# robertknight/ocrs

Measured on AMD Instinct MI355X. Metric: pages/sec end-to-end (1024x1024), higher is better.
Workload: dtype f32

## Files before the change

### ocrs_amd/csrc/kernels_rec.hip

```cpp
#include <algorithm>

#include "common.hpp"
#include "kernels.hpp"
#include "split_mfma.hpp"

namespace ocrs {
namespace k {

typedef float f32x16 __attribute__((ext_vector_type(16)));
typedef unsigned u32x4 __attribute__((ext_vector_type(4)));
typedef float f32x4 __attribute__((ext_vector_type(4)));
typedef float f32x2 __attribute__((ext_vector_type(2)));
typedef unsigned u32x2 __attribute__((ext_vector_type(2)));
typedef __bf16 bf16x8 __attribute__((ext_vector_type(8)));
typedef __bf16 bf16x2 __attribute__((ext_vector_type(2)));

__device__ __forceinline__ int xcd_remap(int b, int nwg) {
    const int xcd = b & 7, q = nwg >> 3, r = nwg & 7;
    return (xcd < r ? xcd * (q + 1) : r * (q + 1) + (xcd - r) * q) + (b >> 3);
}

__device__ __forceinline__ int find_group(const int32_t* __restrict__ toff, int G, int tile) {
    int lo = 0, hi = G;
    while (hi - lo > 1) {
        int mid = (lo + hi) >> 1;
        if (toff[mid] <= tile) lo = mid; else hi = mid;
    }
    return lo;
}

__global__ void __launch_bounds__(256)
conv1_relu_pool_ragged_kernel(const float* __restrict__ x, RaggedView in, const float* __restrict__ wt,
                              const float* __restrict__ bias, int cout, float* __restrict__ y, RaggedView out) {
    __shared__ float sw[9 * 64 + 64];
    for (int i = threadIdx.x; i < 9 * cout; i += 256) sw[i] = wt[i];
    for (int i = threadIdx.x; i < cout; i += 256) sw[9 * 64 + i] = bias[i];
    __syncthreads();
    const int g = find_group(out.toff256, out.G, blockIdx.x);
    const int tile = blockIdx.x - out.toff256[g];
    const int ow = out.W[g], oh = out.H, iw = in.W[g], ih = in.H;
    const int64_t rows = (int64_t)out.n[g] * oh * ow;
    const float* __restrict__ xg = x + in.poff[g];
    float* __restrict__ yg = y + out.poff[g] * cout;
    const int cq = cout >> 2;
    const int step_px = 256 / cq;
    const int q = threadIdx.x % cq;
    int64_t r = (int64_t)tile * 256 + threadIdx.x / cq;
    int ox = (int)(r % ow);
    int64_t t0 = r / ow;
    int oy = (int)(t0 % oh);
    int64_t img = t0 / oh;
    float wq[9][4], bq[4];
#pragma unroll
    for (int t = 0; t < 9; t++)
#pragma unroll
        for (int c = 0; c < 4; c++) wq[t][c] = sw[t * cout + 4 * q + c];
#pragma unroll
    for (int c = 0; c < 4; c++) bq[c] = sw[9 * 64 + 4 * q + c];
    for (int it = 0; it < cq; it++, r += step_px) {
        if (r >= rows) break;
        if (it > 0) {
            ox += step_px;
            while (ox >= ow) { ox -= ow; if (++oy == oh) { oy = 0; img++; } }
        }
        const float* xi = xg + img * ih * iw;
        float p[4][4];
        const int iy0 = 2 * oy - 1, ix0 = 2 * ox - 1;
        if (iy0 >= 0 && iy0 + 3 < ih && ix0 >= 0 && ix0 + 3 < iw) {
            const float* pp = xi + (int64_t)iy0 * iw + ix0;
#pragma unroll
            for (int a = 0; a < 4; a++)
#pragma unroll
                for (int b = 0; b < 4; b++) p[a][b] = pp[a * iw + b];
        } else {
#pragma unroll
            for (int a = 0; a < 4; a++)
#pragma unroll
                for (int b = 0; b < 4; b++) {
                    const int iy = iy0 + a, ix = ix0 + b;
                    p[a][b] = ((unsigned)iy < (unsigned)ih && (unsigned)ix < (unsigned)iw) ? xi[(int64_t)iy * iw + ix] : 0.0f;
                }
        }
        float m[4];
#pragma unroll
        for (int py = 0; py < 2; py++)
#pragma unroll
            for (int px = 0; px < 2; px++) {
                float acc[4];
#pragma unroll
                for (int c = 0; c < 4; c++) acc[c] = bq[c];
#pragma unroll
                for (int ky = 0; ky < 3; ky++)
#pragma unroll
                    for (int kx = 0; kx < 3; kx++) {
                        const float xv = p[py + ky][px + kx];
#pragma unroll
                        for (int c = 0; c < 4; c++) acc[c] = fmaf(xv, wq[ky * 3 + kx][c], acc[c]);
                    }
#pragma unroll
                for (int c = 0; c < 4; c++) {
                    float v = acc[c] > 0.0f ? acc[c] : 0.0f;
                    if (py == 0 && px == 0) m[c] = v;
                    else m[c] = v > m[c] ? v : m[c];
                }
            }
        *reinterpret_cast<float4*>(yg + r * cout + 4 * q) = make_float4(m[0], m[1], m[2], m[3]);
    }
}

void conv1_relu_pool_ragged(const float* x, const RaggedView& in, const float* wt, const float* bias, int cout,
                            float* y, const RaggedView& out, hipStream_t s) {
    if (out.ntiles256 <= 0) return;
    hipLaunchKernelGGL(conv1_relu_pool_ragged_kernel, dim3(out.ntiles256), dim3(256), 0, s, x, in, wt, bias, cout, y, out);
}

template <bool AVG>
__global__ void __launch_bounds__(256)
pool_ragged_kernel(const float* __restrict__ x, RaggedView in, int c, int kh, int kw, float* __restrict__ y,
                   RaggedView out) {
    const int g = find_group(out.toff256, out.G, blockIdx.x);
    const int tile = blockIdx.x - out.toff256[g];
    const int ow = out.W[g], oh = out.H, iw = in.W[g], ih = in.H;
    const int64_t rows = (int64_t)out.n[g] * oh * ow;
    const float* __restrict__ xg = x + in.poff[g] * c;
    float* __restrict__ yg = y + out.poff[g] * c;
    const int cq = c >> 2;
    const float inv = 1.0f / (float)(kh * kw);
    for (int i = threadIdx.x; i < 256 * cq; i += 256) {
        const int64_t r = (int64_t)tile * 256 + i / cq;
        if (r >= rows) break;
        const int q = i % cq;
        const int ox = (int)(r % ow);
        const int oy = (int)((r / ow) % oh);
        const int64_t img = r / ((int64_t)ow * oh);
        const float* xp = xg + ((img * ih + (int64_t)oy * kh) * iw + (int64_t)ox * kw) * c + 4 * q;
        float4 acc = AVG ? make_float4(0.f, 0.f, 0.f, 0.f) : *reinterpret_cast<const float4*>(xp);
        for (int ky = 0; ky < kh; ky++)
            for (int kx = 0; kx < kw; kx++) {
                const float4 v = *reinterpret_cast<const float4*>(xp + ((int64_t)ky * iw + kx) * c);
                if (AVG) { acc.x = acc.x + v.x; acc.y = acc.y + v.y; acc.z = acc.z + v.z; acc.w = acc.w + v.w; }
                else {
                    acc.x = v.x > acc.x ? v.x : acc.x; acc.y = v.y > acc.y ? v.y : acc.y;
                    acc.z = v.z > acc.z ? v.z : acc.z; acc.w = v.w > acc.w ? v.w : acc.w;
                }
            }
        if (AVG) { acc.x = acc.x * inv; acc.y = acc.y * inv; acc.z = acc.z * inv; acc.w = acc.w * inv; }
        *reinterpret_cast<float4*>(yg + r * c + 4 * q) = acc;
    }
}

void pool_ragged(const float* x, const RaggedView& in, int c, int kh, int kw, bool avg, float* y, const RaggedView& out,
                 hipStream_t s) {
    if (out.ntiles256 <= 0) return;
    if (avg) hipLaunchKernelGGL((pool_ragged_kernel<true>), dim3(out.ntiles256), dim3(256), 0, s, x, in, c, kh, kw, y, out);
    else hipLaunchKernelGGL((pool_ragged_kernel<false>), dim3(out.ntiles256), dim3(256), 0, s, x, in, c, kh, kw, y, out);
}

__global__ void __launch_bounds__(256)
to_seq_packed_ragged_kernel(const float* __restrict__ x, RaggedView in, int c, const int32_t* __restrict__ pos,
                            const int32_t* __restrict__ off, float* __restrict__ y) {
    const int g = find_group(in.toff256, in.G, blockIdx.x);
    const int tile = blockIdx.x - in.toff256[g];
    const int T = in.W[g];
    const int64_t rows = (int64_t)in.n[g] * T;
    const float* __restrict__ xg = x + in.poff[g] * c;
    const int32_t* __restrict__ posg = pos + in.loff[g];
    const int cq = c >> 2;
    for (int i = threadIdx.x; i < 256 * cq; i += 256) {
        const int64_t r = (int64_t)tile * 256 + i / cq;
        if (r >= rows) break;
        const int q = i % cq;
        const int t = (int)(r % T);
        const int line = (int)(r / T);
        const float4 v = *reinterpret_cast<const float4*>(xg + r * c + 4 * q);
        *reinterpret_cast<float4*>(y + ((int64_t)off[t] + posg[line]) * c + 4 * q) = v;
    }
}

__global__ void __launch_bounds__(256)
avgpool_to_seq_ragged_kernel(const float* __restrict__ x, RaggedView in, RaggedView seq, int c,
                             const int32_t* __restrict__ pos, const int32_t* __restrict__ off, float* __restrict__ y) {
    const int g = find_group(seq.toff256, seq.G, blockIdx.x);
    const int tile = blockIdx.x - seq.toff256[g];
    const int T = seq.W[g], ih = in.H;
    const int64_t rows = (int64_t)seq.n[g] * T;
    const float* __restrict__ xg = x + in.poff[g] * c;
    const int32_t* __restrict__ posg = pos + seq.loff[g];
    const int cq = c >> 2;
    const float inv = 1.0f / (float)ih;
    for (int i = threadIdx.x; i < 256 * cq; i += 256) {
        const int64_t r = (int64_t)tile * 256 + i / cq;
        if (r >= rows) break;
        const int q = i % cq;
        const int t = (int)(r % T);
        const int64_t line = r / T;
        const float* xp = xg + (line * ih * T + t) * c + 4 * q;
        float4 acc = make_float4(0.f, 0.f, 0.f, 0.f);
        for (int ky = 0; ky < ih; ky++) {
            const float4 v = *reinterpret_cast<const float4*>(xp + (int64_t)ky * T * c);
            acc.x = acc.x + v.x; acc.y = acc.y + v.y; acc.z = acc.z + v.z; acc.w = acc.w + v.w;
        }
        acc.x = acc.x * inv; acc.y = acc.y * inv; acc.z = acc.z * inv; acc.w = acc.w * inv;
        *reinterpret_cast<float4*>(y + ((int64_t)off[t] + posg[line]) * c + 4 * q) = acc;
    }
}

void avgpool_to_seq_ragged(const float* x, const RaggedView& in, const RaggedView& seq, int c, const int32_t* d_pos,
                           const int32_t* d_off, float* y, hipStream_t s) {
    if (seq.ntiles256 <= 0) return;
    hipLaunchKernelGGL(avgpool_to_seq_ragged_kernel, dim3(seq.ntiles256), dim3(256), 0, s, x, in, seq, c, d_pos, d_off, y);
}

void to_seq_packed_ragged(const float* x, const RaggedView& in, int c, const int32_t* d_pos, const int32_t* d_off,
                          float* y, hipStream_t s) {
    if (in.ntiles256 <= 0) return;
    hipLaunchKernelGGL(to_seq_packed_ragged_kernel, dim3(in.ntiles256), dim3(256), 0, s, x, in, c, d_pos, d_off, y);
}

constexpr int RG_BM = 128, RG_BK = 16, RG_LDA = RG_BM + 1;
constexpr int CONV_WAVES = 4;
template <int BN, int TW, int PH, int PW, bool FLAT, int SPLIT = 0>
__global__ void __launch_bounds__(256, SPLIT == 3 ? 2 : SPLIT == 2 ? 3 : CONV_WAVES)
conv3x3_ragged_kernel(const float* __restrict__ X, RaggedView rv, int cin, const float* __restrict__ Bw,
                      const float* __restrict__ bias, int cout, int relu, float* __restrict__ Y,
                      const int64_t* __restrict__ out_poff) {
    extern __shared__ __attribute__((aligned(16))) float lds[];
    constexpr int NTW = BN / 64;
    constexpr int TH = RG_BM / TW;
    static_assert(TW == 32 || TW == 16, "patch width");
    static_assert(!SPLIT || (BN == 128 && RG_BK == 16), "split mode: 128-column blocks, 16-deep chunks");
    constexpr int NP = SPLIT ? SPLIT : 1;
    constexpr int SP_PLANE = split::PLANE;
    float* As = lds;
    float* Bs = lds + (SPLIT ? 2 * NP * SP_PLANE : 2 * RG_BK * RG_LDA);
    const int tid = threadIdx.x, lane = tid & 63, wave = tid >> 6;
    const int half = lane >> 5, l31 = lane & 31;
    const int wm = wave >> 1, wn = wave & 1;
    const int gtile = xcd_remap(blockIdx.x, gridDim.x);
    const int32_t* __restrict__ toff = FLAT ? (PW == 2 ? rv.toff2d_flat2 : rv.toff2d_flat) : rv.toff2d;
    const int g = find_group(toff, rv.G, gtile);
    const int tile = gtile - toff[g];
    const int H = rv.H, W = rv.W[g];
    const int tiles_h = H / TH;
    const int Wp = FLAT ? (PW == 2 ? (W + 1) & ~1 : W) : W;
    const int nimg = FLAT ? rv.n[g] : 1;
    int rb, img, x0, span = 1;
    if (FLAT) {
        rb = tile % tiles_h;
        const int c0 = (tile / tiles_h) * TW;
        img = c0 / Wp;
        x0 = c0 - img * Wp;
        span = min(nimg - img, (x0 + TW - 1) / Wp + 1);
    } else {
        const int tiles_w = (W + TW - 1) / TW;
        const int cb = tile % tiles_w;
        const int t2 = tile / tiles_w;
        rb = t2 % tiles_h;
        img = t2 / tiles_h;
        x0 = cb * TW;
    }
    const int y0 = rb * TH;
    const int n0 = blockIdx.y * BN;
    const float* __restrict__ A = X + (rv.poff[g] + (int64_t)img * H * W) * cin;
    const int K = 9 * cin;

    constexpr int AQ = RG_BK / 4;
    constexpr int AROWS = 256 / AQ;
    constexpr int AV = RG_BM / AROWS;
    const int ar = tid / AQ, akq = tid % AQ;
    int aoff[AV];
    unsigned amask[AV];
#pragma unroll
    for (int j = 0; j < AV; j++) {
        const int m = ar + AROWS * j;
        const int py = y0 + m / TW;
        int px = x0 + m % TW, ir = 0;
        if (FLAT) {
#pragma unroll
            for (int q = 0; q < 3; q++) { const bool nx = px >= Wp; px -= nx ? Wp : 0; ir += nx; }
        }
        unsigned mk = 0;
        if (px < W && ir < span) {
#pragma unroll
            for (int t9 = 0; t9 < 9; t9++) {
                const int iy = py + t9 / 3 - 1, ix = px + t9 % 3 - 1;
                if ((unsigned)iy < (unsigned)H && (unsigned)ix < (unsigned)W) mk |= 1u << t9;
            }
        }
        amask[j] = mk;
        aoff[j] = ((min(ir, span - 1) * H + py) * W + min(px, W - 1)) * cin + akq * 4;
    }
    constexpr int BV = RG_BK * BN / 4 / 256;
    f32x4 pa0[AV], pa1[AV];
    const uint64_t a_addr = reinterpret_cast<uint64_t>(A);
    const float* a_uniform = reinterpret_cast<const float*>(((uint64_t)(uint32_t)__builtin_amdgcn_readfirstlane((int)(a_addr >> 32)) << 32) |
                                                            (uint32_t)__builtin_amdgcn_readfirstlane((int)a_addr));
    const __amdgpu_buffer_rsrc_t a_rsrc = __builtin_amdgcn_make_buffer_rsrc(
        const_cast<float*>(a_uniform),  0,
        __builtin_amdgcn_readfirstlane((int)((int64_t)span * H * W * cin * sizeof(float))), 0x00020000);
    constexpr int OOB = 0x40000000;
    auto load_a_into = [&](int k0, f32x4 (&d0)[AV], f32x4 (&d1)[AV]) {
        const int tap = k0 / cin;
        const int ci0 = k0 - tap * cin;
        const int ky = tap / 3, kx = tap - ky * 3;
        const int delta = ((ky - 1) * W + (kx - 1)) * cin + ci0;
#pragma unroll
        for (int j = 0; j < AV; j++) {
            const int voff = ((amask[j] >> tap) & 1u) ? (aoff[j] + delta) * 4 : OOB;
            const u32x4 v0 = __builtin_amdgcn_raw_buffer_load_b128(a_rsrc, voff, 0, 0);
            const u32x4 v1 = __builtin_amdgcn_raw_buffer_load_b128(a_rsrc, voff + RG_BK * 4, 0, 0);
            d0[j] = __builtin_bit_cast(f32x4, v0);
            d1[j] = __builtin_bit_cast(f32x4, v1);
        }
    };
    auto load_a_pair = [&](int k0) { load_a_into(k0, pa0, pa1); };
    int boff[BV];
#pragma unroll
    for (int j = 0; j < BV; j++) {
        const int idx = tid + 256 * j;
        const int kk = idx / (BN / 4), nn = (idx % (BN / 4)) * 4;
        boff[j] = kk * cout + min(n0 + nn, cout - 4);
    }
    auto load_b = [&](int k0, int buf) {
        if constexpr (SPLIT != 0) {
            split::load_weights<NP>(Bw + ((int64_t)blockIdx.y * (K / RG_BK) + k0 / RG_BK) * split::image_floats,
                                    Bs + buf * NP * SP_PLANE, wave, lane);
            return;
        }
        const float* __restrict__ bk = Bw + (int64_t)k0 * cout;
        float* bdst = Bs + buf * RG_BK * BN + wave * 256;
#pragma unroll
        for (int j = 0; j < BV; j++)
            __builtin_amdgcn_global_load_lds((const __attribute__((address_space(1))) void*)(bk + boff[j]),
                                             (__attribute__((address_space(3))) void*)(bdst + 1024 * j), 16, 0, 0);
    };
    auto commit = [&](int buf, const f32x4 (&pa)[AV]) {
        if constexpr (SPLIT != 0) {
            char* base = reinterpret_cast<char*>(As + buf * NP * SP_PLANE);
#pragma unroll
            for (int j = 0; j < AV; j++) split::commit4<NP>(base, ar + AROWS * j, akq, pa[j][0], pa[j][1], pa[j][2], pa[j][3]);
            return;
        }
        float* a = As + buf * RG_BK * RG_LDA;
#pragma unroll
        for (int j = 0; j < AV; j++) {
            const int r = ar + AROWS * j;
            a[(akq * 4 + 0) * RG_LDA + r] = pa[j].x;
            a[(akq * 4 + 1) * RG_LDA + r] = pa[j].y;
            a[(akq * 4 + 2) * RG_LDA + r] = pa[j].z;
            a[(akq * 4 + 3) * RG_LDA + r] = pa[j].w;
        }
    };

    f32x16 acc[2][NTW];
#pragma unroll
    for (int t = 0; t < NTW; t++) {
        const int col = n0 + wn * (BN / 2) + t * 32 + l31;
        const float bv = col < cout ? bias[col] : 0.0f;
#pragma unroll
        for (int r = 0; r < 16; r++) { acc[0][t][r] = bv; acc[1][t][r] = bv; }
    }
    auto compute = [&](int buf, int bbuf = -1) {
        if constexpr (SPLIT != 0) {
            split::mma_chunk<NP>(reinterpret_cast<const char*>(As + buf * NP * SP_PLANE),
                                 reinterpret_cast<const char*>(Bs + (bbuf < 0 ? buf : bbuf) * NP * SP_PLANE), wm, wn, l31, half, acc);
            return;
        }
        const float* a = As + buf * RG_BK * RG_LDA + wm * 64 + l31;
        const float* b = Bs + buf * RG_BK * BN + wn * (BN / 2) + l31;
#pragma unroll
        for (int kp = 0; kp < RG_BK / 2; kp++) {
            const int kr = 2 * kp + half;
            const float a0 = a[kr * RG_LDA], a1 = a[kr * RG_LDA + 32];
#pragma unroll
            for (int t = 0; t < NTW; t++) {
                const float bt = b[kr * BN + t * 32];
                acc[0][t] = __builtin_amdgcn_mfma_f32_32x32x2f32(a0, bt, acc[0][t], 0, 0, 0);
                acc[1][t] = __builtin_amdgcn_mfma_f32_32x32x2f32(a1, bt, acc[1][t], 0, 0, 0);
            }
        }
    };
    const int nchunks = K / RG_BK;
    if constexpr (SPLIT != 0) {
        static_assert(AV == 2, "split::pipeline counts four activation loads per chunk pair");
        split::pipeline<NP>(nchunks,
                            [&](int k0, f32x4 (&d0)[AV], f32x4 (&d1)[AV]) { load_a_into(k0, d0, d1); },
                            [&](int k0, int ring) { load_b(k0, ring); },
                            [&](int abuf, const f32x4 (&d)[AV]) { commit(abuf, d); },
                            [&](int abuf, int ring) { compute(abuf, ring); });
    } else {
    load_a_pair(0);
    load_b(0, 0);
    commit(0, pa0);
    __syncthreads();
    for (int c = 0; c < nchunks; c += 2) {
        load_b((c + 1) * RG_BK, 1);
        compute(0);
        commit(1, pa1);
        __syncthreads();
        const bool more = c + 2 < nchunks;
        if (more) {
            load_a_pair((c + 2) * RG_BK);
            load_b((c + 2) * RG_BK, 0);
        }
        compute(1);
        if (more) commit(0, pa0);
        __syncthreads();
    }
    }

    const int Ho = H / PH, Wo = W / PW;
    float* __restrict__ C = Y + (out_poff[g] + (int64_t)img * Ho * Wo) * cout;
    auto act = [&](float v) { return relu ? (v > 0.0f ? v : 0.0f) : v; };
    if (PH == 1 && PW == 1 && n0 + BN <= cout && (cout & 3) == 0 && (((uintptr_t)Y) & 15) == 0) {
        constexpr int WN = BN / 2, LPR = WN / 4, RPI = 64 / LPR, NIT = 32 / RPI;
        static_assert(SPLIT != 0 || 4 * 32 * WN <= 2 * RG_BK * RG_LDA + 2 * RG_BK * BN, "staging must fit the operand tiles");
        float* stage = lds + wave * (32 * WN);
        const int srow = lane / LPR, sc4 = (lane % LPR) * 4;
        int soff[NIT];
#pragma unroll
        for (int it = 0; it < NIT; it++) {
            const int q = it * RPI + srow;
            int x = x0 + (TW == 32 ? q : (q & 15)), ir = 0;
            if (FLAT) {
#pragma unroll
                for (int k = 0; k < 3; k++) { const bool nx = x >= Wp; x -= nx ? Wp : 0; ir += nx; }
            }
            soff[it] = (x < W && (!FLAT || ir < span)) ? ((FLAT ? ir * Ho * Wo : 0) + x) * cout + n0 + wn * WN + sc4 : -1;
        }
#pragma unroll
        for (int i = 0; i < 2; i++) {
#pragma unroll
            for (int t = 0; t < NTW; t++)
#pragma unroll
                for (int r = 0; r < 16; r++)
                    stage[((r & 3) + 8 * (r >> 2) + 4 * half) * WN + t * 32 + l31] = act(acc[i][t][r]);
            asm volatile("s_waitcnt lgkmcnt(0)" ::: "memory");
#pragma unroll
            for (int it = 0; it < NIT; it++) {
                const int q = it * RPI + srow;
                if (soff[it] < 0) continue;
                const int ty = TW == 32 ? 2 * wm + i : 4 * wm + 2 * i + (q >> 4);
                *reinterpret_cast<f32x4*>(&C[soff[it] + (y0 + ty) * Wo * cout]) = *reinterpret_cast<const f32x4*>(&stage[q * WN + sc4]);
            }
            asm volatile("s_waitcnt lgkmcnt(0)" ::: "memory");
        }
        return;
    }
    constexpr int NX = TW == 16 ? 8 : 16;
    int xo_off[FLAT ? NX : 1];
    if (FLAT) {
#pragma unroll
        for (int jx = 0; jx < NX; jx++) {
            if (PW == 2 && (jx & 1)) { xo_off[jx] = -1; continue; }
            const int q = (jx & 3) + 8 * (jx >> 2) + 4 * half;
            int x = x0 + (TW == 32 ? q : (q & 15)), ir = 0;
#pragma unroll
            for (int k = 0; k < 3; k++) { const bool nx = x >= Wp; x -= nx ? Wp : 0; ir += nx; }
            xo_off[jx] = (x + (PW - 1) < W && ir < span) ? (ir * Ho * Wo + x / PW) * cout : -1;
        }
    }
#pragma unroll
    for (int t = 0; t < NTW; t++) {
        const int col = n0 + wn * (BN / 2) + t * 32 + l31;
        if (col >= cout) continue;
#pragma unroll
        for (int i = 0; i < 2; i++) {
            if (PH == 2 && TW == 32 && i == 1) continue;
#pragma unroll
            for (int r = 0; r < 16; r++) {
                if (PH == 2 && TW == 16 && (r & 8)) continue;
                if (PW == 2 && (r & 1)) continue;
                const int q = (r & 3) + 8 * (r >> 2) + 4 * half;
                const int ty = TW == 32 ? 2 * wm + i : 4 * wm + 2 * i + (r >> 3);
                const int tx = TW == 32 ? q : (q & 15);
                const int x = x0 + tx;
                if (FLAT ? xo_off[TW == 16 ? (r & 7) : r] < 0 : x + (PW - 1) >= W) continue;
                constexpr int VI = (PH == 2 && TW == 32) ? 1 : 0;
                constexpr int VR = (PH == 2 && TW == 16) ? 8 : 0;
                float m = act(acc[i][t][r]);
                if (PW == 2) { const float v = act(acc[i][t][(r + 1) & 15]); m = v > m ? v : m; }
                if (PH == 2) {
                    { const float v = act(acc[(i + VI) & 1][t][(r + VR) & 15]); m = v > m ? v : m; }
                    if (PW == 2) { const float v = act(acc[(i + VI) & 1][t][(r + VR + 1) & 15]); m = v > m ? v : m; }
                }
                const int yo = (y0 + ty) / PH;
                if (FLAT) C[xo_off[TW == 16 ? (r & 7) : r] + yo * Wo * cout + col] = m;
                else C[((int64_t)yo * Wo + x / PW) * cout + col] = m;
            }
        }
    }
}

constexpr int F12_MID = 32, F12_COUT = 64, F12_TW = 16, F12_TH = 8, F12_HW = F12_TW + 2, F12_HH = F12_TH + 2;
constexpr int F12_NPOS = F12_HH * F12_HW;
constexpr int F12_LD = F12_MID + 1;
constexpr int F12_BK = 16;
constexpr size_t F12_LDS = (size_t)(F12_NPOS * F12_LD + 2 * F12_BK * F12_COUT) * sizeof(float);

__global__ void __launch_bounds__(256, CONV_WAVES)
conv12_fused_kernel(const float* __restrict__ X0, RaggedView in0, RaggedView mid, const float* __restrict__ w1,
                    const float* __restrict__ b1, const float* __restrict__ Bw, const float* __restrict__ bias,
                    float* __restrict__ Y, const int64_t* __restrict__ out_poff) {
    extern __shared__ __attribute__((aligned(16))) float lds[];
    constexpr int BN = F12_COUT, TW = F12_TW, TH = F12_TH, LD = F12_LD;
    float* T = lds;
    float* Bs = lds + F12_NPOS * LD;
    const int tid = threadIdx.x, lane = tid & 63, wave = tid >> 6;
    const int half = lane >> 5, l31 = lane & 31;
    const int wm = wave >> 1, wn = wave & 1;
    const int gtile = xcd_remap(blockIdx.x, gridDim.x);
    const int g = find_group(mid.toff2d_gap, mid.G, gtile);
    const int tile = gtile - mid.toff2d_gap[g];
    const int H = mid.H, W = mid.W[g];
    const int H0 = in0.H, W0 = in0.W[g];
    const int tiles_h = H / TH;
    const int Wg = (W + 2) & ~1;
    const int nimg = mid.n[g];
    const int rb = tile % tiles_h;
    const int c0 = (tile / tiles_h) * TW;
    const int img = c0 / Wg;
    const int x0 = c0 - img * Wg;
    const int span = min(nimg - img, (x0 + TW - 1) / Wg + 1);
    const int y0 = rb * TH;

    constexpr int BV = F12_BK * BN / 4 / 256;
    const int boff = (tid / (BN / 4)) * BN + (tid % (BN / 4)) * 4;
    auto load_b = [&](int k0, int buf) {
#pragma unroll
        for (int j = 0; j < BV; j++)
            __builtin_amdgcn_global_load_lds((const __attribute__((address_space(1))) void*)(Bw + (int64_t)(k0 + 16 * j) * BN + boff),
                                             (__attribute__((address_space(3))) void*)(Bs + buf * F12_BK * BN + wave * 256 + 1024 * j), 16, 0, 0);
    };
    load_b(0, 0);

    {
        const int q = tid & 7;
        f32x2 wq[9][2], bq[2];
#pragma unroll
        for (int t = 0; t < 9; t++)
#pragma unroll
            for (int c = 0; c < 2; c++) wq[t][c] = f32x2{w1[t * F12_MID + 4 * q + 2 * c], w1[t * F12_MID + 4 * q + 2 * c + 1]};
#pragma unroll
        for (int c = 0; c < 2; c++) bq[c] = f32x2{b1[4 * q + 2 * c], b1[4 * q + 2 * c + 1]};
        const float* __restrict__ xg = X0 + in0.poff[g];
        for (int p = tid >> 3; p < F12_NPOS; p += 32) {
            const int hy = p / F12_HW, hx = p - hy * F12_HW;
            const int y = y0 - 1 + hy;
            int x = x0 - 1 + hx, ir = 0;
#pragma unroll
            for (int k = 0; k < 3; k++) { const bool nx = x >= Wg; x -= nx ? Wg : 0; ir += nx; }
            f32x2 m[2] = {f32x2{0.0f, 0.0f}, f32x2{0.0f, 0.0f}};
            if ((unsigned)y < (unsigned)H && x >= 0 && x < W && ir < span) {
                const float* xi = xg + (int64_t)(img + ir) * H0 * W0;
                float pt[4][4];
                const int iy0 = 2 * y - 1, ix0 = 2 * x - 1;
                if (iy0 >= 0 && iy0 + 3 < H0 && ix0 >= 0 && ix0 + 3 < W0) {
                    const float* pp = xi + (int64_t)iy0 * W0 + ix0;
#pragma unroll
                    for (int a = 0; a < 4; a++)
#pragma unroll
                        for (int b = 0; b < 4; b++) pt[a][b] = pp[a * W0 + b];
                } else {
#pragma unroll
                    for (int a = 0; a < 4; a++)
#pragma unroll
                        for (int b = 0; b < 4; b++) {
                            const int iy = iy0 + a, ix = ix0 + b;
                            pt[a][b] = ((unsigned)iy < (unsigned)H0 && (unsigned)ix < (unsigned)W0) ? xi[(int64_t)iy * W0 + ix] : 0.0f;
                        }
                }
#pragma unroll
                for (int py = 0; py < 2; py++)
#pragma unroll
                    for (int px = 0; px < 2; px++) {
                        f32x2 acc[2] = {bq[0], bq[1]};
#pragma unroll
                        for (int ky = 0; ky < 3; ky++)
#pragma unroll
                            for (int kx = 0; kx < 3; kx++) {
                                const float xs = pt[py + ky][px + kx];
                                const f32x2 xv = f32x2{xs, xs};
#pragma unroll
                                for (int c = 0; c < 2; c++) acc[c] = __builtin_elementwise_fma(xv, wq[ky * 3 + kx][c], acc[c]);
                            }
#pragma unroll
                        for (int c = 0; c < 2; c++) m[c] = (py == 0 && px == 0) ? acc[c] : __builtin_elementwise_max(acc[c], m[c]);
                    }
#pragma unroll
                for (int c = 0; c < 2; c++) {
                    m[c].x = m[c].x > 0.0f ? m[c].x : 0.0f;
                    m[c].y = m[c].y > 0.0f ? m[c].y : 0.0f;
                }
            }
            float* t = T + p * LD + 4 * q;
            t[0] = m[0].x; t[1] = m[0].y; t[2] = m[1].x; t[3] = m[1].y;
        }
    }

    f32x16 acc[2];
    {
        const int col = wn * 32 + l31;
        const float bv = bias[col];
#pragma unroll
        for (int r = 0; r < 16; r++) { acc[0][r] = bv; acc[1][r] = bv; }
    }
    int abase[2];
#pragma unroll
    for (int i = 0; i < 2; i++) {
        const int m = wm * 64 + i * 32 + l31;
        abase[i] = ((m / TW) * F12_HW + (m % TW)) * LD + half;
    }
    __syncthreads();
    constexpr int NCH = 9 * F12_MID / F12_BK;
    static_assert(F12_MID % F12_BK == 0 && F12_BK % 16 == 0, "chunk size");
#pragma unroll
    for (int c = 0; c < NCH; c++) {
        if (c + 1 < NCH) load_b((c + 1) * F12_BK, (c + 1) & 1);
        const int tap = (c * F12_BK) / F12_MID, ch0 = (c * F12_BK) % F12_MID;
        const int toff = ((tap / 3) * F12_HW + tap % 3) * LD + ch0;
        const float* b = Bs + (c & 1) * F12_BK * BN + wn * 32 + l31;
#pragma unroll
        for (int kp = 0; kp < F12_BK / 2; kp++) {
            const float a0 = T[abase[0] + toff + 2 * kp], a1 = T[abase[1] + toff + 2 * kp];
            const float bt = b[(2 * kp + half) * BN];
            acc[0] = __builtin_amdgcn_mfma_f32_32x32x2f32(a0, bt, acc[0], 0, 0, 0);
            acc[1] = __builtin_amdgcn_mfma_f32_32x32x2f32(a1, bt, acc[1], 0, 0, 0);
        }
        __syncthreads();
    }

    const int Ho = H / 2, Wo = W / 2;
    float* __restrict__ C = Y + (out_poff[g] + (int64_t)img * Ho * Wo) * BN;
    auto act = [&](float v) { return v > 0.0f ? v : 0.0f; };
    const int col = wn * 32 + l31;
    int xo_off[8];
#pragma unroll
    for (int jx = 0; jx < 8; jx++) {
        if (jx & 1) { xo_off[jx] = -1; continue; }
        int x = x0 + (jx & 3) + 8 * (jx >> 2) + 4 * half, ir = 0;
#pragma unroll
        for (int k = 0; k < 3; k++) { const bool nx = x >= Wg; x -= nx ? Wg : 0; ir += nx; }
        xo_off[jx] = (x + 1 < W && ir < span) ? (ir * Ho * Wo + x / 2) * BN : -1;
    }
#pragma unroll
    for (int i = 0; i < 2; i++)
#pragma unroll
        for (int r = 0; r < 8; r += 2) {
            if (xo_off[r & 7] < 0) continue;
            const float m = act(__builtin_fmaxf(__builtin_fmaxf(acc[i][r], acc[i][r + 1]), __builtin_fmaxf(acc[i][r + 8], acc[i][r + 9])));
            const int yo = (y0 + 4 * wm + 2 * i) / 2;
            C[xo_off[r & 7] + yo * Wo * BN + col] = m;
        }
}

constexpr int F12S_RS = 20;
constexpr int F12S_TILE = F12_HH * F12S_RS * 64;
constexpr int F12S_BTAP = F12_COUT * 64;
constexpr size_t f12s_lds(int np) { return (size_t)np * (F12S_TILE + 3 * F12S_BTAP); }

template <int NP>
__global__ void __launch_bounds__(256, NP == 3 ? 2 : 3)
conv12_fused_split_kernel(const float* __restrict__ X0, RaggedView in0, RaggedView mid, const float* __restrict__ w1,
                          const float* __restrict__ b1, const uint16_t* __restrict__ Bimg, const float* __restrict__ bias,
                          float* __restrict__ Y, const int64_t* __restrict__ out_poff) {
    extern __shared__ __attribute__((aligned(16))) float lds[];
    constexpr int BN = F12_COUT, TW = F12_TW, TH = F12_TH;
    char* T = reinterpret_cast<char*>(lds);
    char* Bs = T + NP * F12S_TILE;
    const int tid = threadIdx.x, lane = tid & 63, wave = tid >> 6;
    const int half = lane >> 5, l31 = lane & 31;
    const int wm = wave >> 1, wn = wave & 1;
    const int gtile = xcd_remap(blockIdx.x, gridDim.x);
    const int g = find_group(mid.toff2d_gap, mid.G, gtile);
    const int tile = gtile - mid.toff2d_gap[g];
    const int H = mid.H, W = mid.W[g];
    const int H0 = in0.H, W0 = in0.W[g];
    const int tiles_h = H / TH;
    const int Wg = (W + 2) & ~1;
    const int nimg = mid.n[g];
    const int rb = tile % tiles_h;
    const int c0 = (tile / tiles_h) * TW;
    const int img = c0 / Wg;
    const int x0 = c0 - img * Wg;
    const int span = min(nimg - img, (x0 + TW - 1) / Wg + 1);
    const int y0 = rb * TH;

    auto load_b = [&](int tap) {
        const char* src = reinterpret_cast<const char*>(Bimg) + (size_t)tap * 3 * F12S_BTAP;
        char* dst = Bs + (tap % 3) * NP * F12S_BTAP;
#pragma unroll
        for (int p = 0; p < NP; p++)
            __builtin_amdgcn_global_load_lds((const __attribute__((address_space(1))) void*)(src + p * F12S_BTAP + wave * 1024 + lane * 16),
                                             (__attribute__((address_space(3))) void*)(dst + p * F12S_BTAP + wave * 1024), 16, 0, 0);
    };
    load_b(0);
    load_b(1);

    {
        const int q = tid & 7;
        f32x2 wq[9][2], bq[2];
#pragma unroll
        for (int t = 0; t < 9; t++)
#pragma unroll
            for (int c = 0; c < 2; c++) wq[t][c] = f32x2{w1[t * F12_MID + 4 * q + 2 * c], w1[t * F12_MID + 4 * q + 2 * c + 1]};
#pragma unroll
        for (int c = 0; c < 2; c++) bq[c] = f32x2{b1[4 * q + 2 * c], b1[4 * q + 2 * c + 1]};
        const float* __restrict__ xg = X0 + in0.poff[g];
        auto cut = [](float a, float b) { return __builtin_bit_cast(unsigned, __builtin_convertvector(f32x2{a, b}, bf16x2)); };
        auto lo_f = [](unsigned pk) { return __uint_as_float(pk << 16); };
        auto hi_f = [](unsigned pk) { return __uint_as_float(pk & 0xFFFF0000u); };
        for (int p = tid >> 3; p < F12_NPOS; p += 32) {
            const int hy = p / F12_HW, hx = p - hy * F12_HW;
            const int y = y0 - 1 + hy;
            int x = x0 - 1 + hx, ir = 0;
#pragma unroll
            for (int k = 0; k < 3; k++) { const bool nx = x >= Wg; x -= nx ? Wg : 0; ir += nx; }
            f32x2 m[2] = {f32x2{0.0f, 0.0f}, f32x2{0.0f, 0.0f}};
            if ((unsigned)y < (unsigned)H && x >= 0 && x < W && ir < span) {
                const float* xi = xg + (int64_t)(img + ir) * H0 * W0;
                float pt[4][4];
                const int iy0 = 2 * y - 1, ix0 = 2 * x - 1;
                if (iy0 >= 0 && iy0 + 3 < H0 && ix0 >= 0 && ix0 + 3 < W0) {
                    const float* pp = xi + (int64_t)iy0 * W0 + ix0;
#pragma unroll
                    for (int a = 0; a < 4; a++)
#pragma unroll
                        for (int b = 0; b < 4; b++) pt[a][b] = pp[a * W0 + b];
                } else {
#pragma unroll
                    for (int a = 0; a < 4; a++)
#pragma unroll
                        for (int b = 0; b < 4; b++) {
                            const int iy = iy0 + a, ix = ix0 + b;
                            pt[a][b] = ((unsigned)iy < (unsigned)H0 && (unsigned)ix < (unsigned)W0) ? xi[(int64_t)iy * W0 + ix] : 0.0f;
                        }
                }
#pragma unroll
                for (int py = 0; py < 2; py++)
#pragma unroll
                    for (int px = 0; px < 2; px++) {
                        f32x2 acc[2] = {bq[0], bq[1]};
#pragma unroll
                        for (int ky = 0; ky < 3; ky++)
#pragma unroll
                            for (int kx = 0; kx < 3; kx++) {
                                const float xs = pt[py + ky][px + kx];
                                const f32x2 xv = f32x2{xs, xs};
#pragma unroll
                                for (int c = 0; c < 2; c++) acc[c] = __builtin_elementwise_fma(xv, wq[ky * 3 + kx][c], acc[c]);
                            }
#pragma unroll
                        for (int c = 0; c < 2; c++) m[c] = (py == 0 && px == 0) ? acc[c] : __builtin_elementwise_max(acc[c], m[c]);
                    }
#pragma unroll
                for (int c = 0; c < 2; c++) {
                    m[c].x = m[c].x > 0.0f ? m[c].x : 0.0f;
                    m[c].y = m[c].y > 0.0f ? m[c].y : 0.0f;
                }
            }
            const int off = (hy * F12S_RS + hx) * 64 + ((((q >> 1) ^ (hx >> 2)) & 3) << 4) + ((q & 1) << 3);
            u32x2 ph = {cut(m[0].x, m[0].y), cut(m[1].x, m[1].y)};
            const float r0 = m[0].x - lo_f(ph[0]), r1 = m[0].y - hi_f(ph[0]), r2 = m[1].x - lo_f(ph[1]), r3 = m[1].y - hi_f(ph[1]);
            u32x2 pm = {cut(r0, r1), cut(r2, r3)};
            *reinterpret_cast<u32x2*>(T + off) = ph;
            *reinterpret_cast<u32x2*>(T + F12S_TILE + off) = pm;
            if (NP == 3) {
                u32x2 pl = {cut(r0 - lo_f(pm[0]), r1 - hi_f(pm[0])), cut(r2 - lo_f(pm[1]), r3 - hi_f(pm[1]))};
                *reinterpret_cast<u32x2*>(T + 2 * F12S_TILE + off) = pl;
            }
        }
    }

    f32x16 acc[2];
    {
        const float bv = bias[wn * 32 + l31];
#pragma unroll
        for (int r = 0; r < 16; r++) { acc[0][r] = bv; acc[1][r] = bv; }
    }
    const int mx = l31 & 15;
    int pos0[2];
#pragma unroll
    for (int i = 0; i < 2; i++) {
        const int m = wm * 64 + i * 32 + l31;
        pos0[i] = (m / TW) * F12S_RS + mx;
    }
    const int nb = wn * 32 + l31;
    const int boff = nb * 64, bsw = (nb >> 2) & 3;
    asm volatile("" ::: "memory");
    __builtin_amdgcn_s_waitcnt(0x0070);
    __builtin_amdgcn_s_barrier();
    asm volatile("" ::: "memory");
#pragma unroll
    for (int tap = 0; tap < 9; tap++) {
        if (tap + 2 < 9) load_b(tap + 2);
        const int ky = tap / 3, kx = tap % 3;
        const int asw = ((mx + kx) >> 2) & 3;
        const char* bb = Bs + (tap % 3) * NP * F12S_BTAP + boff;
#pragma unroll
        for (int s2 = 0; s2 < 2; s2++) {
            const int qa = (((2 * s2 + half) ^ asw) & 3) << 4, qb = (((2 * s2 + half) ^ bsw) & 3) << 4;
            bf16x8 af[2][3], bfr[3];
#pragma unroll
            for (int i = 0; i < 2; i++)
#pragma unroll
                for (int p = 0; p < NP; p++) af[i][p] = *reinterpret_cast<const bf16x8*>(T + p * F12S_TILE + (pos0[i] + ky * F12S_RS + kx) * 64 + qa);
#pragma unroll
            for (int p = 0; p < NP; p++) bfr[p] = *reinterpret_cast<const bf16x8*>(bb + p * F12S_BTAP + qb);
#define OCRS_TERM12(PA, PB)                                                                                   \
            OCRS_SPLIT_MMA(af[0][PA], bfr[PB], acc[0]);                                                       \
            OCRS_SPLIT_MMA(af[1][PA], bfr[PB], acc[1]);
            if (NP == 3) { OCRS_TERM12(NP - 1, 0) OCRS_TERM12(0, NP - 1) OCRS_TERM12(1, 1) }
            OCRS_TERM12(1, 0) OCRS_TERM12(0, 1) OCRS_TERM12(0, 0)
#undef OCRS_TERM12
        }
        asm volatile("" ::: "memory");
        if (tap + 2 < 9) __builtin_amdgcn_s_waitcnt(0x0070 | NP);
        else __builtin_amdgcn_s_waitcnt(0x0070);
        __builtin_amdgcn_s_barrier();
        asm volatile("" ::: "memory");
    }

    const int Ho = H / 2, Wo = W / 2;
    float* __restrict__ C = Y + (out_poff[g] + (int64_t)img * Ho * Wo) * BN;
    auto act = [&](float v) { return v > 0.0f ? v : 0.0f; };
    const int col = wn * 32 + l31;
    int xo_off[8];
#pragma unroll
    for (int jx = 0; jx < 8; jx++) {
        if (jx & 1) { xo_off[jx] = -1; continue; }
        int x = x0 + (jx & 3) + 8 * (jx >> 2) + 4 * half, ir = 0;
#pragma unroll
        for (int k = 0; k < 3; k++) { const bool nx = x >= Wg; x -= nx ? Wg : 0; ir += nx; }
        xo_off[jx] = (x + 1 < W && ir < span) ? (ir * Ho * Wo + x / 2) * BN : -1;
    }
#pragma unroll
    for (int i = 0; i < 2; i++)
#pragma unroll
        for (int r = 0; r < 8; r += 2) {
            if (xo_off[r & 7] < 0) continue;
            const float m = act(__builtin_fmaxf(__builtin_fmaxf(acc[i][r], acc[i][r + 1]), __builtin_fmaxf(acc[i][r + 8], acc[i][r + 9])));
            const int yo = (y0 + 4 * wm + 2 * i) / 2;
            C[xo_off[r & 7] + yo * Wo * BN + col] = m;
        }
}

void conv12_split_weights(const float* w, std::vector<uint16_t>* out) {
    out->assign((size_t)9 * 3 * F12_COUT * 32, 0);
    auto bits = [](float f) { uint32_t u; memcpy(&u, &f, 4); return u; };
    auto from = [](uint32_t u) { float f; memcpy(&f, &u, 4); return f; };
    auto rne = [&](float f) { const uint32_t u = bits(f); return (u + 0x7FFFu + ((u >> 16) & 1u)) >> 16; };
    for (int tap = 0; tap < 9; tap++)
        for (int n = 0; n < F12_COUT; n++)
            for (int k = 0; k < 32; k++) {
                const float x = w[(size_t)(tap * 32 + k) * F12_COUT + n];
                const uint32_t hb = rne(x);
                const float r1 = x - from(hb << 16);
                const uint32_t mb = rne(r1);
                const uint32_t lb = rne(r1 - from(mb << 16));
                const size_t e = (size_t)n * 32 + (size_t)((((k >> 3) ^ (n >> 2)) & 3) * 8) + (k & 7);
                uint16_t* img = out->data() + (size_t)tap * 3 * F12_COUT * 32;
                img[e] = (uint16_t)hb;
                img[F12_COUT * 32 + e] = (uint16_t)mb;
                img[2 * F12_COUT * 32 + e] = (uint16_t)lb;
            }
}

bool conv12_fused_ragged(const float* x, const RaggedView& in0, const RaggedView& mid, const float* w1, const float* b1,
                         int c1, const float* w2, const float* b2, int c2, float* y, const RaggedView& out, hipStream_t s,
                         const uint16_t* w2split) {
    if (option(OPT_CONV12_FUSE) == 0) return false;
    if (c1 != F12_MID || c2 != F12_COUT || mid.H % F12_TH != 0 || in0.H != 2 * mid.H || out.H * 2 != mid.H) return false;
    if (mid.min_w < 11 || mid.ntiles2d_gap <= 0) return false;
    if (mid.max_tile_px_ * 4 * (int64_t)sizeof(float) >= (int64_t)1 << 30 ||
        mid.max_tile_px_ * F12_COUT * (int64_t)sizeof(float) >= (int64_t)1 << 30) return false;
    if (!x) return true;
    const int numerics = option(OPT_NUMERICS);
    if (numerics != 0 && w2split) {
        static std::atomic<uint64_t> ok3{0}, ok2{0};
        if (numerics == 2) {
            allow_dynamic_lds(reinterpret_cast<const void*>(&conv12_fused_split_kernel<2>), ok2);
            hipLaunchKernelGGL((conv12_fused_split_kernel<2>), dim3(mid.ntiles2d_gap), dim3(256), f12s_lds(2), s, x, in0, mid, w1, b1, w2split, b2, y, out.poff);
        } else {
            allow_dynamic_lds(reinterpret_cast<const void*>(&conv12_fused_split_kernel<3>), ok3);
            hipLaunchKernelGGL((conv12_fused_split_kernel<3>), dim3(mid.ntiles2d_gap), dim3(256), f12s_lds(3), s, x, in0, mid, w1, b1, w2split, b2, y, out.poff);
        }
        return true;
    }
    hipLaunchKernelGGL(conv12_fused_kernel, dim3(mid.ntiles2d_gap), dim3(256), F12_LDS, s, x, in0, mid, w1, b1, w2, b2, y, out.poff);
    return true;
}

void split_weights(const float* w, int K, int N, int ldw, std::vector<uint16_t>* out) {
    const int nblk = N / 128, nch = K / 16;
    out->assign((size_t)nblk * nch * 3 * 128 * 16, 0);
    auto bits = [](float f) { uint32_t u; memcpy(&u, &f, 4); return u; };
    auto from = [](uint32_t u) { float f; memcpy(&f, &u, 4); return f; };
    auto rne = [&](float f) { const uint32_t u = bits(f); return (u + 0x7FFFu + ((u >> 16) & 1u)) >> 16; };
    for (int nb = 0; nb < nblk; nb++)
        for (int c = 0; c < nch; c++) {
            uint16_t* img = out->data() + ((size_t)nb * nch + c) * 3 * 128 * 16;
            for (int n = 0; n < 128; n++)
                for (int kl = 0; kl < 16; kl++) {
                    const float x = w[(size_t)(c * 16 + kl) * ldw + nb * 128 + n];
                    const uint32_t hb = rne(x);
                    const float r1 = x - from(hb << 16);
                    const uint32_t mb = rne(r1);
                    const uint32_t lb = rne(r1 - from(mb << 16));
                    const int half = kl >> 3, j = kl & 7;
                    const size_t e = (size_t)n * 16 + (size_t)(((half ^ (n >> 3)) & 1) * 8) + j;
                    img[e] = (uint16_t)hb;
                    img[128 * 16 + e] = (uint16_t)mb;
                    img[2 * 128 * 16 + e] = (uint16_t)lb;
                }
        }
}

bool conv3x3_ragged(const float* x, const RaggedView& rv, int cin, const float* wt, const float* bias, int cout, int relu,
                    int ph, int pw, float* y, const RaggedView& out, hipStream_t s, const uint16_t* wsplit) {
    if ((cin % (2 * RG_BK)) != 0 || (cout % 4) != 0 || cout < 64) return false;
    if (!((ph == 1 && pw == 1) || (ph == 2 && (pw == 1 || pw == 2)))) return false;
    if ((ph == 2 || pw == 2) && !relu) return false;
    if (rv.tw != 32 && rv.tw != 16) return false;
    if (rv.H % (RG_BM / rv.tw) != 0) return false;
    const bool flat = option(OPT_CONV_FLAT) != 0 && rv.min_w >= 11 &&
                      rv.max_tile_px_ * std::max(cin, cout) * (int64_t)sizeof(float) < (int64_t)1 << 30;
    if (!flat && (int64_t)rv.H * rv.max_w * cin * (int64_t)sizeof(float) >= (int64_t)1 << 30) return false;
    const int ntiles = flat ? (pw == 2 ? rv.ntiles2d_flat2 : rv.ntiles2d_flat) : rv.ntiles2d;
    if (ntiles <= 0) return true;
    const bool n64 = cout <= 64;
    const int numerics = option(OPT_NUMERICS);
    const bool split = wsplit && !n64 && (cout % 128) == 0 && (cin % 64) == 0 && numerics != 0;
    const size_t lds = split ? split::lds_bytes(numerics == 2 ? 2 : 3)
                             : (size_t)(2 * RG_BK * RG_LDA + 2 * RG_BK * (n64 ? 64 : 128)) * sizeof(float);
    const dim3 grid(ntiles, (cout + (n64 ? 63 : 127)) / (n64 ? 64 : 128));
#define OCRS_LAUNCH_SPLIT(TW_, PH_, PW_, FLAT_, NP_, SLOT_)                                                              \
    if (flat == FLAT_ && (numerics == 2 ? 2 : 3) == NP_) {                                                              \
        allow_dynamic_lds(reinterpret_cast<const void*>(&conv3x3_ragged_kernel<128, TW_, PH_, PW_, FLAT_, NP_>), ok_[SLOT_]);   \
        hipLaunchKernelGGL((conv3x3_ragged_kernel<128, TW_, PH_, PW_, FLAT_, NP_>), grid, dim3(256), lds, s, x, rv, cin, ws_, bias, \
                           cout, relu, y, out.poff);                                                                    \
    }
#define OCRS_LAUNCH_CONV(BN_, TW_, PH_, PW_)                                                                            \
    do {                                                                                                                \
        if (split && BN_ == 128) {                                                                                      \
            const float* ws_ = reinterpret_cast<const float*>(wsplit);                                                  \
            static std::atomic<uint64_t> ok_[4] = {};                                                                    \
            OCRS_LAUNCH_SPLIT(TW_, PH_, PW_, true, 3, 0) OCRS_LAUNCH_SPLIT(TW_, PH_, PW_, false, 3, 1)                     \
            OCRS_LAUNCH_SPLIT(TW_, PH_, PW_, true, 2, 2) OCRS_LAUNCH_SPLIT(TW_, PH_, PW_, false, 2, 3)                     \
        } else if (flat) hipLaunchKernelGGL((conv3x3_ragged_kernel<BN_, TW_, PH_, PW_, true>), grid, dim3(256), lds, s, x, rv, \
                                     cin, wt, bias, cout, relu, y, out.poff);                                           \
        else hipLaunchKernelGGL((conv3x3_ragged_kernel<BN_, TW_, PH_, PW_, false>), grid, dim3(256), lds, s, x, rv,     \
                                cin, wt, bias, cout, relu, y, out.poff);                                                \
    } while (0)
#define OCRS_DISPATCH_POOL(BN_, TW_)                              \
    do {                                                          \
        if (ph == 1) OCRS_LAUNCH_CONV(BN_, TW_, 1, 1);            \
        else if (pw == 1) OCRS_LAUNCH_CONV(BN_, TW_, 2, 1);       \
        else OCRS_LAUNCH_CONV(BN_, TW_, 2, 2);                    \
    } while (0)
    if (n64) {
        if (rv.tw == 32) OCRS_DISPATCH_POOL(64, 32); else OCRS_DISPATCH_POOL(64, 16);
    } else {
        if (rv.tw == 32) OCRS_DISPATCH_POOL(128, 32); else OCRS_DISPATCH_POOL(128, 16);
    }
#undef OCRS_DISPATCH_POOL
#undef OCRS_LAUNCH_CONV
#undef OCRS_LAUNCH_SPLIT
    return true;
}

}
}
```

Measured before the change: 267.6.

## Add LDS halo-window conv3x3 kernel for cin=64 flat recognition layers

Adds a new 3x3 convolution kernel for cin=64 layers in the flat ragged path. It loads the whole input halo window (tile plus a one-pixel border, all 64 channels) into LDS once and runs the nine taps as shifted reads from that window, instead of re-staging im2col tiles for every K chunk. Weights are prefetched from registers via buffer loads in a double-buffered pipeline, and the unpooled case stores output through LDS staging as vectorized writes. Tiles are split in half to keep enough workgroups, at the cost of a larger per-block LDS footprint and less reuse of weight loads across the tile.

```diff
diff --git a/ocrs_amd/csrc/kernels_rec.hip b/ocrs_amd/csrc/kernels_rec.hip
--- a/ocrs_amd/csrc/kernels_rec.hip
+++ b/ocrs_amd/csrc/kernels_rec.hip
@@ -492,6 +492,203 @@
     }
 }
 
+constexpr int WN_TW = 16, WN_TH = 4, WN_HW = WN_TW + 2, WN_HH = WN_TH + 2, WN_BN = 128, WN_BK = 16;
+constexpr int wn_ldc(int cin) { return cin + 1; }
+constexpr int wn_row(int cin) { return WN_HW * wn_ldc(cin) + ((16 - WN_HW * wn_ldc(cin)) % 32 + 32) % 32; }
+constexpr int wn_win_floats(int cin) { return (WN_HH * wn_row(cin) + cin + 3) & ~3; }
+constexpr int WN_THREADS = 256;
+constexpr size_t wn_lds(int cin) {
+    return (size_t)std::max(wn_win_floats(cin), WN_THREADS / 64 * 64 * 32) * sizeof(float);
+}
+
+template <int CIN, int PH, int PW>
+__global__ void __launch_bounds__(WN_THREADS, 2)
+conv3x3_window_kernel(const float* __restrict__ X, RaggedView rv, const float* __restrict__ Bw,
+                      const float* __restrict__ bias, int cout, int relu, float* __restrict__ Y,
+                      const int64_t* __restrict__ out_poff) {
+    extern __shared__ __attribute__((aligned(16))) float lds[];
+    constexpr int LDC = wn_ldc(CIN), WROW = wn_row(CIN), ZOFF = WN_HH * WROW;
+    constexpr int BN = WN_BN, TW = WN_TW, WCOL = BN / 4;
+    static_assert(LDC % 32 == 1 && WROW % 32 == 16, "bank-conflict-free operand reads");
+    static_assert(4 * 64 * WCOL * sizeof(float) <= wn_lds(CIN), "epilogue staging must fit");
+    float* T = lds;
+    const int tid = threadIdx.x, lane = tid & 63, wave = tid >> 6;
+    const int half = lane >> 5, l31 = lane & 31;
+    const int wn = wave;
+    const int gtile = xcd_remap(blockIdx.x, gridDim.x);
+    const int ptile = gtile >> 1, sub = gtile & 1;
+    const int32_t* __restrict__ toff = PW == 2 ? rv.toff2d_flat2 : rv.toff2d_flat;
+    const int g = find_group(toff, rv.G, ptile);
+    const int tile = ptile - toff[g];
+    const int H = rv.H, W = rv.W[g];
+    const int ptw = rv.tw, tiles_h = H / (128 / ptw);
+    const int Wp = PW == 2 ? (W + 1) & ~1 : W;
+    const int nimg = rv.n[g];
+    const int rb = tile % tiles_h;
+    const int c0 = (tile / tiles_h) * ptw + (ptw == 32 ? sub * TW : 0);
+    const int y0 = ptw == 32 ? rb * WN_TH : rb * 8 + sub * WN_TH;
+    const int img = c0 / Wp;
+    if (img >= nimg) return;
+    const int x0 = c0 - img * Wp;
+    const int span = min(nimg - img, (x0 + TW - 1) / Wp + 1);
+    const int n0 = blockIdx.y * BN;
+    const float* __restrict__ A = X + (rv.poff[g] + (int64_t)img * H * W) * CIN;
+    constexpr int K = 9 * CIN, NCH = K / WN_BK;
+
+    const __amdgpu_buffer_rsrc_t b_rsrc = __builtin_amdgcn_make_buffer_rsrc(const_cast<float*>(Bw),  0,
+                                                                            K * cout * (int)sizeof(float), 0x00020000);
+    const int bvoff = (half * cout + n0 + wn * WCOL + l31) * (int)sizeof(float);
+    auto load_b = [&](int c, float (&d)[WN_BK / 2]) {
+#pragma unroll
+        for (int kp = 0; kp < WN_BK / 2; kp++)
+            d[kp] = __builtin_bit_cast(float, __builtin_amdgcn_raw_buffer_load_b32(b_rsrc, bvoff, (c * WN_BK + 2 * kp) * cout * (int)sizeof(float), 0));
+    };
+    float p0[WN_BK / 2], p1[WN_BK / 2], q0[WN_BK / 2], q1[WN_BK / 2];
+    load_b(0, p0);
+    load_b(1, p1);
+
+    {
+        constexpr int CQ = CIN / 4, NITEM = WN_HH * WN_HW * CQ, NIT = (NITEM + WN_THREADS - 1) / WN_THREADS;
+        const uint64_t a_addr = reinterpret_cast<uint64_t>(A);
+        const float* a_uniform = reinterpret_cast<const float*>(((uint64_t)(uint32_t)__builtin_amdgcn_readfirstlane((int)(a_addr >> 32)) << 32) |
+                                                                (uint32_t)__builtin_amdgcn_readfirstlane((int)a_addr));
+        const __amdgpu_buffer_rsrc_t a_rsrc = __builtin_amdgcn_make_buffer_rsrc(
+            const_cast<float*>(a_uniform),  0,
+            __builtin_amdgcn_readfirstlane((int)((unsigned)min(nimg - img, 3) * H * W * CIN * sizeof(float))), 0x00020000);
+        constexpr unsigned OOB = 0xFFFFFFF0u;
+        f32x4 v[NIT];
+#pragma unroll
+        for (int j = 0; j < NIT; j++) {
+            const int it = tid + WN_THREADS * j;
+            const int p = it / CQ, q = it % CQ;
+            const int hy = p / WN_HW, hx = p - hy * WN_HW;
+            const int y = y0 - 1 + hy;
+            int x = x0 - 1 + hx, ir = 0;
+#pragma unroll
+            for (int k = 0; k < 3; k++) { const bool nx = x >= Wp; x -= nx ? Wp : 0; ir += nx; }
+            const bool in = it < NITEM && (unsigned)y < (unsigned)H && x >= 0 && x < W && ir < nimg - img;
+            v[j] = __builtin_bit_cast(f32x4, __builtin_amdgcn_raw_buffer_load_b128(
+                       a_rsrc, in ? (unsigned)((((ir * H + y) * W + x) * CIN + 4 * q) * 4) : OOB, 0, 0));
+        }
+#pragma unroll
+        for (int j = 0; j < NIT; j++) {
+            const int it = tid + WN_THREADS * j;
+            if (it >= NITEM) continue;
+            const int p = it / CQ, q = it % CQ;
+            const int hy = p / WN_HW, hx = p - hy * WN_HW;
+            float* t = T + hy * WROW + hx * LDC + 4 * q;
+            t[0] = v[j].x; t[1] = v[j].y; t[2] = v[j].z; t[3] = v[j].w;
+        }
+        if (tid < CIN) T[ZOFF + tid] = 0.0f;
+    }
+
+    int abase[2][9];
+    {
+        const int px = l31 & 15;
+        int x = x0 + px, ir = 0;
+#pragma unroll
+        for (int k = 0; k < 3; k++) { const bool nx = x >= Wp; x -= nx ? Wp : 0; ir += nx; }
+        const bool valid = x < W && ir < span;
+#pragma unroll
+        for (int i = 0; i < 2; i++)
+#pragma unroll
+            for (int t9 = 0; t9 < 9; t9++) {
+                const int ky = t9 / 3, kx = t9 % 3, py = 2 * i + (l31 >> 4);
+                const bool in = valid && x + kx - 1 >= 0 && x + kx - 1 < W;
+                abase[i][t9] = (in ? (py + ky) * WROW + (px + kx) * LDC : ZOFF) + half;
+            }
+    }
+
+    f32x16 acc[2];
+    {
+        const float bv = bias[n0 + wn * WCOL + l31];
+#pragma unroll
+        for (int r = 0; r < 16; r++) { acc[0][r] = bv; acc[1][r] = bv; }
+    }
+    auto compute = [&](int aoff0, int aoff1, const float (&b)[WN_BK / 2]) {
+#pragma unroll
+        for (int kp = 0; kp < WN_BK / 2; kp++) {
+            const float a0 = T[aoff0 + 2 * kp], a1 = T[aoff1 + 2 * kp];
+            acc[0] = __builtin_amdgcn_mfma_f32_32x32x2f32(a0, b[kp], acc[0], 0, 0, 0);
+            acc[1] = __builtin_amdgcn_mfma_f32_32x32x2f32(a1, b[kp], acc[1], 0, 0, 0);
+        }
+    };
+    __syncthreads();
+#pragma unroll
+    for (int tap = 0; tap < 9; tap++) {
+        const int ab0 = abase[0][tap], ab1 = abase[1][tap];
+#pragma unroll 1
+        for (int cc = 0; cc < CIN / WN_BK; cc += 4) {
+            const int c = tap * (CIN / WN_BK) + cc;
+            load_b(min(c + 2, NCH - 1), q0);
+            load_b(min(c + 3, NCH - 1), q1);
+            asm volatile("" ::: "memory");
+            compute(ab0 + cc * WN_BK, ab1 + cc * WN_BK, p0);
+            compute(ab0 + (cc + 1) * WN_BK, ab1 + (cc + 1) * WN_BK, p1);
+            load_b(min(c + 4, NCH - 1), p0);
+            load_b(min(c + 5, NCH - 1), p1);
+            asm volatile("" ::: "memory");
+            compute(ab0 + (cc + 2) * WN_BK, ab1 + (cc + 2) * WN_BK, q0);
+            compute(ab0 + (cc + 3) * WN_BK, ab1 + (cc + 3) * WN_BK, q1);
+        }
+    }
+
+    const int Ho = H / PH, Wo = W / PW;
+    float* __restrict__ C = Y + (out_poff[g] + (int64_t)img * Ho * Wo) * cout;
+    auto act = [&](float v) { return relu ? (v > 0.0f ? v : 0.0f) : v; };
+    if (PH == 1 && PW == 1 && (((uintptr_t)Y) & 15) == 0) {
+        constexpr int WN = WCOL, LPR = WN / 4, RPI = 64 / LPR, NIT = 64 / RPI;
+        __syncthreads();
+        float* stage = lds + wave * (64 * WN);
+        const int srow = lane / LPR, sc4 = (lane % LPR) * 4;
+#pragma unroll
+        for (int i = 0; i < 2; i++)
+#pragma unroll
+            for (int r = 0; r < 16; r++)
+                stage[(i * 32 + (r & 3) + 8 * (r >> 2) + 4 * half) * WN + l31] = act(acc[i][r]);
+        asm volatile("s_waitcnt lgkmcnt(0)" ::: "memory");
+#pragma unroll
+        for (int it = 0; it < NIT; it++) {
+            const int q = it * RPI + srow;
+            int x = x0 + (q & 15), ir = 0;
+#pragma unroll
+            for (int k = 0; k < 3; k++) { const bool nx = x >= Wp; x -= nx ? Wp : 0; ir += nx; }
+            if (x >= W || ir >= span) continue;
+            const int ty = q >> 4;
+            *reinterpret_cast<f32x4*>(&C[((ir * Ho + y0 + ty) * Wo + x) * cout + n0 + wn * WN + sc4]) =
+                *reinterpret_cast<const f32x4*>(&stage[q * WN + sc4]);
+        }
+        return;
+    }
+    int xo_off[8];
+#pragma unroll
+    for (int jx = 0; jx < 8; jx++) {
+        if (PW == 2 && (jx & 1)) { xo_off[jx] = -1; continue; }
+        int x = x0 + (jx & 3) + 8 * (jx >> 2) + 4 * half, ir = 0;
+#pragma unroll
+        for (int k = 0; k < 3; k++) { const bool nx = x >= Wp; x -= nx ? Wp : 0; ir += nx; }
+        xo_off[jx] = (x + (PW - 1) < W && ir < span) ? (ir * Ho * Wo + x / PW) * cout : -1;
+    }
+    const int col = n0 + wn * WCOL + l31;
+#pragma unroll
+    for (int i = 0; i < 2; i++) {
+#pragma unroll
+        for (int r = 0; r < 16; r++) {
+            if (PH == 2 && (r & 8)) continue;
+            if (PW == 2 && (r & 1)) continue;
+            if (xo_off[r & 7] < 0) continue;
+            float m = act(acc[i][r]);
+            if (PW == 2) { const float v = act(acc[i][(r + 1) & 15]); m = v > m ? v : m; }
+            if (PH == 2) {
+                { const float v = act(acc[i][(r + 8) & 15]); m = v > m ? v : m; }
+                if (PW == 2) { const float v = act(acc[i][(r + 9) & 15]); m = v > m ? v : m; }
+            }
+            const int yo = (y0 + 2 * i + (r >> 3)) / PH;
+            C[xo_off[r & 7] + yo * Wo * cout + col] = m;
+        }
+    }
+}
+
 constexpr int F12_MID = 32, F12_COUT = 64, F12_TW = 16, F12_TH = 8, F12_HW = F12_TW + 2, F12_HH = F12_TH + 2;
 constexpr int F12_NPOS = F12_HH * F12_HW;
 constexpr int F12_LD = F12_MID + 1;
@@ -933,6 +1130,27 @@
     const bool split = wsplit && !n64 && (cout % 128) == 0 && (cin % 64) == 0 && numerics != 0;
     const size_t lds = split ? split::lds_bytes(numerics == 2 ? 2 : 3)
                              : (size_t)(2 * RG_BK * RG_LDA + 2 * RG_BK * (n64 ? 64 : 128)) * sizeof(float);
+    if (flat && !split && cin == 64 && (cout % WN_BN) == 0 &&
+        (int64_t)3 * rv.H * rv.max_w * cin * (int64_t)sizeof(float) < (int64_t)1 << 31) {
+        const dim3 wgrid(2 * ntiles, cout / WN_BN);
+#define OCRS_LAUNCH_WINDOW(CIN_, PH_, PW_)                                                                              \
+        do {                                                                                                            \
+            static std::atomic<uint64_t> okw_{0};                                                                       \
+            allow_dynamic_lds(reinterpret_cast<const void*>(&conv3x3_window_kernel<CIN_, PH_, PW_>), okw_);             \
+            hipLaunchKernelGGL((conv3x3_window_kernel<CIN_, PH_, PW_>), wgrid, dim3(WN_THREADS), wn_lds(CIN_), s, x, rv, wt, bias, \
+                               cout, relu, y, out.poff);                                                                \
+        } while (0)
+#define OCRS_WINDOW_POOL(CIN_)                                              \
+        do {                                                                \
+            if (ph == 1) OCRS_LAUNCH_WINDOW(CIN_, 1, 1);                    \
+            else if (pw == 1) OCRS_LAUNCH_WINDOW(CIN_, 2, 1);               \
+            else OCRS_LAUNCH_WINDOW(CIN_, 2, 2);                            \
+        } while (0)
+        OCRS_WINDOW_POOL(64);
+#undef OCRS_WINDOW_POOL
+#undef OCRS_LAUNCH_WINDOW
+        return true;
+    }
     const dim3 grid(ntiles, (cout + (n64 ? 63 : 127)) / (n64 ? 64 : 128));
 #define OCRS_LAUNCH_SPLIT(TW_, PH_, PW_, FLAT_, NP_, SLOT_)                                                              \
     if (flat == FLAT_ && (numerics == 2 ? 2 : 3) == NP_) {                                                              \
```

After: 273.3, median of 6. 1.02x the previous value.
